# jaymarichua/Applestar

Hardware: AMD Instinct MI355X
Metric: learner samples/sec (AlphaStar policy) (higher is better)
Workload: dtype fp32

## Files before the change

applestar_amd/csrc/bindings.cpp:

```cpp
#include <cstring>
#include <cstdlib>
#include <map>
#include <string>
#include <torch/extension.h>
#include <c10/hip/HIPStream.h>
#include <c10/hip/HIPGuard.h>

#include "kernels.h"

namespace {

hipStream_t stream() { return c10::hip::getCurrentHIPStream().stream(); }

int dt(const at::Tensor& t) {
  if (t.scalar_type() == at::kFloat) return as::DT_F32;
  if (t.scalar_type() == at::kBFloat16) return as::DT_BF16;
  TORCH_CHECK(false, "applestar_amd: unsupported dtype ", t.scalar_type());
}

void check_cuda(const at::Tensor& t, const char* name) {
  TORCH_CHECK(t.is_cuda(), "applestar_amd: ", name, " must be a GPU tensor");
  TORCH_CHECK(t.is_contiguous(), "applestar_amd: ", name, " must be contiguous");
}

// ... 1467 lines not shown
  }
  c10::hip::HIPGuard g(dy.device().index());
  auto opts = out_bf16 ? dy.options() : dy.options().dtype(at::kFloat);
  auto dw = at::empty({N, K}, opts);
  at::Tensor db = want_bias ? at::empty({N}, opts) : at::Tensor();
  if (R == 0) {
    dw.zero_();
    if (want_bias) db.zero_();
    return {dw, db};
  }
  as::small_tn(dy.data_ptr(), x.data_ptr(), mp, static_cast<int>(mask_mode), dw.data_ptr(),
               want_bias ? db.data_ptr() : nullptr, R, static_cast<int>(N), static_cast<int>(K), bf, out_bf16, stream());
  return {dw, db};
}

std::vector<at::Tensor> wgrad_f32(const at::Tensor& dy, const at::Tensor& x, int64_t cin, bool want_bias,
                                  const c10::optional<at::Tensor>& out) {
  check_cuda(dy, "dy");
  check_cuda(x, "x");
  TORCH_CHECK(dy.scalar_type() == at::kFloat && x.scalar_type() == at::kFloat, "wgrad_f32: fp32 dy / x");
  TORCH_CHECK(dy.dim() == 2 && dy.is_contiguous() && x.is_contiguous(), "wgrad_f32: contiguous dy [R, N], x");
  const int64_t R = dy.size(0), N = dy.size(1);
  int64_t K, H = 1, W = 1;
  if (cin > 0) {
    TORCH_CHECK(x.dim() == 4 && x.size(3) == cin && x.size(0) * x.size(1) * x.size(2) == R, "wgrad_f32: x NHWC");
    H = x.size(1);
    W = x.size(2);
    K = 9 * cin;
    TORCH_CHECK(cin % 4 == 0, "wgrad_f32: Cin % 4");
  } else {
    TORCH_CHECK(x.dim() == 2 && x.size(0) == R, "wgrad_f32: x [R, K]");
    K = x.size(1);
  }
  TORCH_CHECK(N % 4 == 0 && K % 4 == 0, "wgrad_f32: N and K must be multiples of 4");
  TORCH_CHECK(R * N * 4 < 0x7ffffff0LL && x.numel() * 4 < 0x7ffffff0LL, "wgrad_f32: tensor too large");
  c10::hip::HIPGuard g(dy.device().index());
  auto opts = dy.options();
  const int64_t NK = N * K, stride = NK + (want_bias ? N : 0);
  at::Tensor flat;
  if (out && out->defined()) {
    TORCH_CHECK(out->scalar_type() == at::kFloat && out->is_contiguous() && out->numel() == stride &&
                out->device() == dy.device(), "wgrad_f32: out must be a contiguous fp32 [N K (+ N)] buffer");
    flat = *out;
  }
  if (R == 0) {
    if (flat.defined()) {
      flat.zero_();
      return {flat.narrow(0, 0, NK).view({N, K}), want_bias ? flat.narrow(0, NK, N) : at::Tensor()};
    }
    return {at::zeros({N, K}, opts), want_bias ? at::zeros({N}, opts) : at::Tensor()};
  }
  const int S = cin > 0 ? as::conv_wgrad_f32_splits(R, static_cast<int>(N), static_cast<int>(K), static_cast<int>(H),
                                                    static_cast<int>(W), static_cast<int>(cin))
                        : as::wgrad_f32_splits(R, static_cast<int>(N), static_cast<int>(K));
  auto part = (S == 1 && flat.defined()) ? flat.view({1, stride}) : at::empty({S, stride}, opts);
  as::wgrad_f32(dy.data_ptr<float>(), x.data_ptr<float>(), part.data_ptr<float>(),
                want_bias ? part.data_ptr<float>() + NK : nullptr, stride, R, static_cast<int>(N), static_cast<int>(K),
                static_cast<int>(H), static_cast<int>(W), static_cast<int>(cin), S, stream());
  if (S == 1) {
    if (!flat.defined()) flat = part.view({stride});
  } else {
    if (!flat.defined()) flat = at::empty({stride}, opts);
    as::column_reduce(part.data_ptr<float>(), flat.data_ptr<float>(), S, static_cast<int>(stride), stream());
  }
  return {flat.narrow(0, 0, NK).view({N, K}), want_bias ? flat.narrow(0, NK, N) : at::Tensor()};
}

std::vector<at::Tensor> wgrad(const at::Tensor& dy, const at::Tensor& x, int64_t cin, bool want_bias, bool bf16_out) {
  check_cuda(dy, "dy");
  check_cuda(x, "x");
  TORCH_CHECK(dy.scalar_type() == at::kBFloat16 && x.scalar_type() == at::kBFloat16, "wgrad: bf16 dy / x");
  TORCH_CHECK(dy.dim() == 2, "wgrad: dy [R, N]");
  TORCH_CHECK(dy.is_contiguous() && x.is_contiguous(), "wgrad: dy and x must be contiguous");
  const int64_t R = dy.size(0), N = dy.size(1);
  int64_t K, H = 1, W = 1;
  if (cin > 0) {
    TORCH_CHECK(x.dim() == 4 && x.size(3) == cin && x.size(0) * x.size(1) * x.size(2) == R, "wgrad: x NHWC");
    H = x.size(1);
    W = x.size(2);
    K = 9 * cin;
    TORCH_CHECK(cin % 8 == 0, "wgrad: Cin % 8");
  } else {
    TORCH_CHECK(x.dim() == 2 && x.size(0) == R, "wgrad: x [R, K]");
    K = x.size(1);
  }
  TORCH_CHECK(N % 8 == 0 && K % 8 == 0, "wgrad: N and K must be multiples of 8");
  TORCH_CHECK(R * N * 2 < 0x7ffffff0LL && x.numel() * 2 < 0x7ffffff0LL, "wgrad: tensor too large");
  c10::hip::HIPGuard g(dy.device().index());
  const int S = R > 0 ? as::wgrad_splits(R, static_cast<int>(N), static_cast<int>(K)) : 1;
  auto opts = dy.options().dtype(at::kFloat);
  if (R == 0) {
    auto zo = bf16_out ? dy.options() : opts;
    return {at::zeros({N, K}, zo), want_bias ? at::zeros({N}, zo) : at::Tensor()};
  }
  const int64_t NK = N * K, stride = NK + (want_bias ? N : 0);
  if (bf16_out && S == 1) {
    auto flat = at::empty({stride}, dy.options());
    as::wgrad(dy.data_ptr(), x.data_ptr(), reinterpret_cast<float*>(flat.data_ptr()),
              want_bias ? reinterpret_cast<float*>(static_cast<at::BFloat16*>(flat.data_ptr()) + NK) : nullptr, 0, R,
              static_cast<int>(N), static_cast<int>(K), static_cast<int>(H), static_cast<int>(W), static_cast<int>(cin),
              1, stream(), true);
    return {flat.narrow(0, 0, NK).view({N, K}), want_bias ? flat.narrow(0, NK, N) : at::Tensor()};
  }
  auto part = at::empty({S, stride}, opts);
  static const bool nan_fill = [] {
    const char* e = std::getenv("APPLESTAR_WGRAD_NANFILL");
    return e != nullptr && e[0] == '1';
// ... 758 lines not shown
  }
  flush();
}

at::Tensor pointwise_conv(const at::Tensor& x, const at::Tensor& w, const c10::optional<at::Tensor>& bias, int64_t act) {
  check_cuda(x, "x");
  check_cuda(w, "w");
  TORCH_CHECK(x.scalar_type() == at::kBFloat16 && x.dim() == 2, "pointwise: x [P, cin] bf16");
  TORCH_CHECK(w.scalar_type() == at::kFloat && w.dim() == 2 && w.size(1) == x.size(1), "pointwise: w fp32 [cout, cin]");
  const int64_t P = x.size(0), cin = x.size(1), cout = w.size(0);
  TORCH_CHECK(as::pointwise_supported(static_cast<int>(cin), static_cast<int>(cout)), "pointwise: channels");
  const float* bp = nullptr;
  if (bias.has_value()) {
    check_cuda(*bias, "bias");
    TORCH_CHECK(bias->scalar_type() == at::kFloat && bias->numel() == cout, "pointwise: bias fp32 [cout]");
    bp = bias->data_ptr<float>();
  }
  c10::hip::HIPGuard g(x.device().index());
  auto y = at::empty({P, cout}, x.options());
  as::pointwise_conv(x.data_ptr(), w.data_ptr<float>(), bp, y.data_ptr(), P, static_cast<int>(cin),
                     static_cast<int>(cout), static_cast<int>(act), stream());
  return y;
}

void register_codec(pybind11::module& m);

PYBIND11_MODULE(TORCH_EXTENSION_NAME, m) {
  m.doc() = "applestar_amd HIP kernels for gfx950 (MI355X)";
  register_codec(m);
  m.def("layer_norm_fwd", &layer_norm_fwd);
  m.def("layer_norm_bwd", &layer_norm_bwd, py::arg("dy"), py::arg("xin"), py::arg("y"), py::arg("w"), py::arg("mean"),
        py::arg("rstd"), py::arg("dx_dtype"), py::arg("act"), py::arg("mask_src") = py::none());
  m.def("reverse_scan", &reverse_scan);
  m.def("col_sum", &col_sum);
  m.def("multi_logp", &multi_logp);
  m.def("presplit_b", &presplit_b, py::arg("b"), py::arg("trans") = false, py::arg("out") = py::none());
  m.def("gemm_f32_psb_supported", &gemm_f32_psb_supported);
  m.def("multi_presplit", &multi_presplit);
  m.def("conv3x3_f32_psb_supported", &conv3x3_f32_psb_supported);
  m.def("conv3x3_f32_psb", &conv3x3_f32_psb, py::arg("x"), py::arg("wsplit"), py::arg("Cout"),
        py::arg("bias") = py::none(), py::arg("res") = py::none(), py::arg("res2") = py::none(),
        py::arg("mask") = py::none(), py::arg("act") = 0);
  m.def("conv3x3_f32_v2", &conv3x3_f32_v2, py::arg("x"), py::arg("wsplit"), py::arg("Cout"),
        py::arg("bias") = py::none(), py::arg("res") = py::none(), py::arg("res2") = py::none(),
        py::arg("mask") = py::none(), py::arg("act") = 0, py::arg("variant") = 0);
  m.def("conv3x3_f32_halo_supported", &conv3x3_f32_halo_supported);
  m.def("conv3x3_f32_halo", &conv3x3_f32_halo, py::arg("x"), py::arg("wsplit"), py::arg("Cout"),
        py::arg("bias") = py::none(), py::arg("res") = py::none(), py::arg("res2") = py::none(),
        py::arg("mask") = py::none(), py::arg("act") = 0);
  m.def("conv_halo_f32_mode", &as::conv_halo_f32_mode);
  m.def("set_conv_halo_f32_mode", &as::set_conv_halo_f32_mode);
  m.def("conv_wgrad_halo_f32_mode", &as::conv_wgrad_halo_f32_mode);
  m.def("set_conv_wgrad_halo_f32_mode", &as::set_conv_wgrad_halo_f32_mode);
  m.def("conv_wgrad_f32_halo_selected", &as::conv_wgrad_f32_halo_selected, py::arg("cout"), py::arg("h"), py::arg("w"),
        py::arg("cin"));
  m.def("gemm_f32_psb", &gemm_f32_psb, py::arg("a"), py::arg("bsplit"), py::arg("N"), py::arg("K"),
        py::arg("bias") = py::none(), py::arg("res") = py::none(), py::arg("act") = 0, py::arg("variant") = 0);
  m.def("entity_pack", &entity_pack);
  m.def("embed_relu_fwd", &embed_relu_fwd);
  m.def("embed_relu_bwd", &embed_relu_bwd, py::arg("dout"), py::arg("out"), py::arg("idx"), py::arg("V"),
        py::arg("ordered") = false);
  m.def("gated_residual_fwd", &gated_residual_fwd, py::arg("y"), py::arg("g"), py::arg("sp"), py::arg("x"),
        py::arg("post") = py::none());
  m.def("gated_residual_bwd", &gated_residual_bwd, py::arg("dout"), py::arg("y"), py::arg("g"), py::arg("sp"),
        py::arg("out"), py::arg("xin") = py::none());
  m.def("lnlstm_fwd", &lnlstm_fwd, py::arg("xp"), py::arg("h0"), py::arg("c0"), py::arg("wT"),
        py::arg("lnh_w"), py::arg("lnh_b"), py::arg("lnc_w"), py::arg("lnc_b"),
        py::arg("eps"), py::arg("want_bf16") = false);
  m.def("lnlstm_bwd", &lnlstm_bwd);
  m.def("entity_embed_fwd", &entity_embed_fwd);
  m.def("entity_onehot", &entity_onehot);
  m.def("upsample2x_fwd", &upsample2x_fwd);
  m.def("upsample2x_bwd", &upsample2x_bwd, py::arg("dy"), py::arg("mask") = py::none());
  m.def("entity_embed_wgrad", &entity_embed_wgrad);
  m.def("mm_k32", &mm_k32);
  m.def("spatial_embed_fwd", &spatial_embed_fwd, py::arg("planes"), py::arg("effects"), py::arg("w_dense"),
        py::arg("bias"), py::arg("rows"), py::arg("ex"), py::arg("ey"), py::arg("entity_num"), py::arg("out_dtype"),
        py::arg("ordered") = false);
  m.def("spatial_gather_rows", &spatial_gather_rows, py::arg("dpre"), py::arg("ex"), py::arg("ey"),
        py::arg("entity_num"), py::arg("N"), py::arg("gate") = py::none());
  m.def("spatial_dense_input", &spatial_dense_input);
  m.def("spatial_dense_wgrad", &spatial_dense_wgrad, py::arg("planes"), py::arg("effects"), py::arg("dpre"),
        py::arg("gate") = py::none());
  m.def("varlen_attn_fwd", &varlen_attn_fwd);
  m.def("varlen_attn_bwd", &varlen_attn_bwd);
  m.def("varlen_attn_fwd_f32", &varlen_attn_fwd_f32);
  m.def("conv3x3_f32_epi2", &conv3x3_f32_epi2);
  m.def("conv3x3_f32_epi2_supported", &conv3x3_f32_epi2_supported);
  m.def("conv3x3_f32", &conv3x3_f32);
  m.def("fused_clip_adam", &fused_clip_adam);
  m.def("head_sample", &head_sample);
  m.def("target_unit_sample", &target_unit_sample);
  m.def("fused_adam_chunk", &as::fused_adam_chunk);
  m.def("wgrad_f32", &wgrad_f32, py::arg("dy"), py::arg("x"), py::arg("cin"), py::arg("want_bias"),
        py::arg("out") = py::none());
  m.def("gemm_f32", &gemm_f32);
  m.def("gemm_bf16_small", &gemm_bf16_small);
  m.def("gemm_bf16", &gemm_bf16);
  m.def("small_gemm", &small_gemm);
  m.def("small_wgrad", &small_wgrad);
  m.def("small_gemm_splitk", &small_gemm_splitk);
  m.def("f32_mfma_mode", &as::f32_mfma_mode);
  m.def("set_f32_pipe_variant", &as::set_f32_pipe_variant);
  m.def("set_f32_conv_variant", &as::set_f32_conv_variant);
  m.def("set_f32_mfma_mode", &as::set_f32_mfma_mode);
  m.def("conv3x3_f32_supported", &as::conv3x3_f32_supported);
// ... 61 lines not shown
```

applestar_amd/csrc/kernels.h:

```cpp
#pragma once
#include <hip/hip_runtime.h>
#include <stdint.h>

namespace as {

enum DType : int { DT_F32 = 0, DT_BF16 = 1 };
enum SrcType : int { SRC_U8 = 0, SRC_I8 = 1, SRC_I16 = 2, SRC_I32 = 3, SRC_I64 = 4, SRC_F16 = 5, SRC_F32 = 6 };
enum FieldKind : int { FIELD_ONE_HOT = 0, FIELD_BINARY = 1, FIELD_SCALAR = 2 };

constexpr int kMaxFields = 40;
struct EntityFields {
  const void* ptr[kMaxFields];
  int dtype[kMaxFields];
  int kind[kMaxFields];
  int offset[kMaxFields];
  int width[kMaxFields];
  int n;
};

void layer_norm_fwd(const void* x, int x_dt, const void* res, int res_dt, const float* w, const float* b,
                    void* y, int y_dt, float* xsum, float* mean, float* rstd, long rows, int cols, float eps,
                    int act, hipStream_t s);
void layer_norm_bwd(const void* dy, int dy_dt, const void* xin, int xin_dt, const void* y, int y_dt,
                    const float* w, const float* mean, const float* rstd, void* dx, int dx_dt,
// ... 127 lines not shown

namespace as {
void maxpool2_fwd(const void* x, void* y, uint8_t* pos, int dt, int B, int H, int W, int C, hipStream_t s);
void maxpool2_bwd(const void* dy, const uint8_t* pos, void* dx, int dt, int B, int H, int W, int C, hipStream_t s,
                  const void* mask = nullptr);
void maxpool2_bwd_relu(const void* dy, const uint8_t* pos, const void* y, void* dx, int B, int H, int W, int C,
                       hipStream_t s, bool f32 = false);
void segment_sum(const void* x, int dt, const int* cu, float* out, int S, int C, hipStream_t s);
void entity_mean_pool(const void* x, int dt, const bool* valid, const void* num, bool num64, void* out, int B, int N,
                      int C, hipStream_t s);
int ln_affine_slices(long R);
void ln_affine_grads(const float* dy, const float* xh, float* part, long R, int C, hipStream_t s);
void table_grad(const void* src, int dt, const int64_t* idx, float* out, long U, int V, int D, hipStream_t s);

bool conv3x3_supported(int Cin, int Cout);
void conv3x3_fwd(const void* x, const void* w, const float* bias, const void* res, void* out, int B, int H, int W,
                 int Cin, int Cout, int act, hipStream_t s);

bool conv3x3_f32_supported(int Cin, int Cout);
void conv3x3_f32_fwd(const float* x, const float* w, const float* bias, const float* res, float* out, int B, int H,
                     int W, int Cin, int Cout, int act, hipStream_t s);
bool conv3x3_f32_epi2_supported(int Cin, int Cout);
void conv3x3_f32_fwd_epi2(const float* x, const float* w, const float* res, const float* res2, long res2_rows,
                          const float* mask, float* out, int B, int H, int W, int Cin, int Cout, hipStream_t s);
int wgrad_f32_splits(long R, int N, int K);
void set_f32_pipe_variant(int v);
int f32_conv_variant();
void set_f32_conv_variant(int v);
int f32_mfma_mode();
void set_f32_mfma_mode(int mode);
void small_nt(const void* a, const void* b, const float* bias, const void* res, const void* amask, int mask_mode,
              void* out, long M, int N, int K, int act, bool bf16, hipStream_t s);
int small_nt_splits(long M, int N, int K);
void small_nt_splitk(const void* a, const void* b, const float* bias, float* part, int S, void* out, long M, int N,
                     int K, int act, bool bf16, hipStream_t s);
void small_tn(const void* dy, const void* x, const void* ymask, int mask_mode, void* dw, void* db, long R, int N,
              int K, bool bf16_in, bool bf16_out, hipStream_t s);
void gemm_bf16_small(const void* a, const void* b, const float* bias, const void* res, void* out, long M, int N, int K,
                     int act, hipStream_t s);
bool gemm_f32_is_small(long M, int N);
void gemm_bf16(const void* a, const void* b, const float* bias, const void* res, void* out, long M, int N, int K,
               int act, hipStream_t s);
void gemm_f32(const float* a, const float* b, const float* bias, const float* res, float* out, long M, int N, int K,
              int act, hipStream_t s);
void wgrad_f32(const float* dy, const float* x, float* dw_part, float* db_part, long part_stride, long R, int N, int K,
               int H, int W, int Cin, int S, hipStream_t st);
int conv_wgrad_halo_f32_mode();
void set_conv_wgrad_halo_f32_mode(int mode);
bool conv_wgrad_f32_halo_supported(int N, int H, int W, int Cin);
bool conv_wgrad_f32_halo_selected(int N, int H, int W, int Cin);
int conv_wgrad_f32_splits(long R, int N, int K, int H, int W, int Cin);
void conv_wgrad_f32_halo(const float* dy, const float* x, float* dw_part, float* db_part, long part_stride, long R,
                         int N, int K, int H, int W, int Cin, int S, long rows_per_split, hipStream_t st);

void head_sample(const void* logits, int logits_dt, long ld_logits, int B, int C, float inv_t, const uint8_t* mask,
                 long mask_ld, const int64_t* lens, const float* u, const void* table, int table_dt,
                 const float* tbias, int D, float* out_logits, int64_t* action, float* emb, hipStream_t s);
void target_unit_sample(const void* e, int e_dt, const float* w1, const float* b1, const float* w2, const float* b2,
                        const void* key, int key_dt, int B, int N, const int64_t* lens, float inv_t, const float* u,
                        float* out_logits, int64_t* action, hipStream_t s);

int fused_adam_chunk();
void fused_clip_adam(const void* table, const long* chunks, int nchunks, int ntensors, float* part,
                     const float* gate, float* norm_out, float max_norm, float* mom, float* scale, float* mom_init,
                     const float* hp, float lr_bc1, float b1, float b2, float inv_sqrt_bc2, float eps, float wd,
                     int decoupled, hipStream_t s);

int wgrad_splits(long R, int N, int K);

constexpr int kCopyMaxT = 64;
constexpr long kCopyChunk = 8192;
constexpr long kCopyRawChunk = 16384;
struct CopyArgs {
  int ntensors;
  int chunk_start[kCopyMaxT + 1];
  const void* src[kCopyMaxT];
  void* dst[kCopyMaxT];
  long n[kCopyMaxT];
  unsigned char dts[kCopyMaxT];
};
void multi_copy(const CopyArgs& a, hipStream_t s);

constexpr int kColMaxP = 32;
struct ColSumArgs {
  int npieces;
  long rows;
  int block_start[kColMaxP + 1];
  float* dst[kColMaxP];
  int dld[kColMaxP], doff[kColMaxP], width[kColMaxP], nsrc[kColMaxP];
  const float* src[kColMaxP][3];
  int sld[kColMaxP][3], soff[kColMaxP][3];
};
void col_sum(const ColSumArgs& a, hipStream_t s);

constexpr int kLogpMaxH = 8;
struct LogpArgs {
  int nheads;
  long row_start[kLogpMaxH + 1];
  const void* logits[kLogpMaxH];
  const int64_t* action[kLogpMaxH];
  float* out[kLogpMaxH];
  int cols[kLogpMaxH];
  unsigned char bf16[kLogpMaxH];
  long blk_start[kLogpMaxH + 1];
  unsigned char big[kLogpMaxH];
};
// ... 170 lines not shown
```

applestar_amd/csrc/kernels/conv_wgrad_f32_halo.hip:

```cpp
#include <cstdlib>

#include "../common.h"
#include "../kernels.h"
#include "../split_mfma.h"
#include "../f32_pipe.h"
#include "../conv_tap.h"

namespace as {
namespace {

using pipe::f16v;

constexpr int kWgBN = 128, kWgCC = 32, kWgRS = 16, kWgMaxW = 80;

typedef short s16x4 __attribute__((ext_vector_type(4)));
typedef __attribute__((address_space(3))) s16x4 lds_s16x4;

template <int WMAX>
struct WgHaloCfg {
  static constexpr int SA = kWgBN * 2 + 64, SX = kWgCC * 2;
  static constexpr int NRING = 2 * kWgRS + 2 * WMAX + 2 <= 128 ? 128 : 256;
  static constexpr int PA = kWgRS * SA;
  static constexpr int PX = (NRING + 1) * SX;
  static constexpr int SMEM = 6 * PA + 3 * PX;
  static_assert(2 * kWgRS + 2 * WMAX + 2 <= NRING && 2 * SMEM <= 160 * 1024, "ring size / two workgroups per CU");
};

__device__ __forceinline__ s16x4 tr_read(const char* p) {
  return __builtin_amdgcn_ds_read_tr16_b64_v4i16((lds_s16x4*)p);
}

__device__ __forceinline__ u32v4 tr_frag(const char* p0, const char* p1) {
  const uint2 lo = __builtin_bit_cast(uint2, tr_read(p0)), hi = __builtin_bit_cast(uint2, tr_read(p1));
  return u32v4{lo.x, lo.y, hi.x, hi.y};
}

__device__ __forceinline__ void split_store(char* plane0, int plane_bytes, int off, const uint4 v) {
  uint2 s0, s1, s2;
  split4(v, s0, s1, s2);
  *reinterpret_cast<uint2*>(plane0 + off) = s0;
  *reinterpret_cast<uint2*>(plane0 + plane_bytes + off) = s1;
  *reinterpret_cast<uint2*>(plane0 + 2 * plane_bytes + off) = s2;
}

template <int WMAX>
__global__ __launch_bounds__(256, 2) void conv_wgrad_f32_halo_kernel(const float* __restrict__ dy,
                                                                     const float* __restrict__ x,
                                                                     float* __restrict__ dw_part,
                                                                     float* __restrict__ db_part, long part_stride,
                                                                     long R, int N, int K, int H, int W, int Cin,
                                                                     long rows_per_split, int tiles_n, int chunks) {
  using C = WgHaloCfg<WMAX>;
  constexpr int RS = kWgRS, BN = kWgBN, CC = kWgCC, SA = C::SA, SX = C::SX;
  constexpr int RINGB = C::NRING * SX;
  __shared__ __attribute__((aligned(16))) char smem[C::SMEM];
  char* const pa = smem;
  char* const px = smem + 6 * C::PA;

  const int wg = pipe::xcd_remap();
  const int ch = wg % chunks;
  const int tn = (wg / chunks) % tiles_n;
  const int s = wg / (chunks * tiles_n);
  const int n0 = tn * BN, c0 = ch * CC;
  const long r_begin = static_cast<long>(s) * rows_per_split;
  const long r_end = r_begin + rows_per_split < R ? r_begin + rows_per_split : R;
  const int tid = threadIdx.x, lane = tid & 63, wid = __builtin_amdgcn_readfirstlane(tid >> 6);
  const int l32 = lane & 31, h = lane >> 5;
  const int HW = H * W;
  const __amdgpu_buffer_rsrc_t yr =
      __builtin_amdgcn_make_buffer_rsrc(const_cast<float*>(dy), 0, static_cast<int>(R * N * 4), 0x00020000);
  const __amdgpu_buffer_rsrc_t xr =
      __builtin_amdgcn_make_buffer_rsrc(const_cast<float*>(x), 0, static_cast<int>(R * Cin * 4), 0x00020000);
  const int nrows = r_end > r_begin ? static_cast<int>(r_end - r_begin) : 0;
  const int nsteps = (nrows + RS - 1) / RS;

  const int a_q = tid & 31, a_row = tid >> 5;
  const bool a_colok = n0 + 4 * a_q < N;
  int a_base[2], a_lim[2];
#pragma unroll
  for (int i = 0; i < 2; ++i) {
    a_base[i] = static_cast<int>(((r_begin + a_row + 8 * i) * N + n0 + 4 * a_q) * 4);
    a_lim[i] = a_colok ? nrows - (a_row + 8 * i) : 0;
  }
  const int a_step = RS * N * 4;
  const int x_q = tid & 7, x_row = (tid >> 3) & 15;
  const bool x_colok = c0 + 4 * x_q < Cin, x_wave = wid < 2;
  const int x_base = static_cast<int>(((r_begin + W + 1 + x_row) * Cin + c0 + 4 * x_q) * 4);
  const long x_left = R - (r_begin + W + 1 + x_row);
  const int x_lim = (x_colok && x_wave && x_left > 0) ? static_cast<int>(x_left) : 0;
  const int x_step = RS * Cin * 4;
  const bool do_bias = db_part != nullptr && ch == 0;
  const int b_col = n0 + (tid & 127), b_h = tid >> 7;
  const int b_base = static_cast<int>(((r_begin + 8 * b_h) * N + b_col) * 4);
  const int b_lim = b_col < N ? nrows - 8 * b_h : 0;
  float rb[8], bsum = 0.f;
  uint4 ra[2], rx;
// ... 432 lines not shown
```

applestar_amd/csrc/kernels/wgrad_f32.hip:

```cpp
#include "../common.h"
#include "../kernels.h"
#include "../split_mfma.h"
#include "../f32_pipe.h"

namespace as {
namespace {

typedef __attribute__((ext_vector_type(16))) float f16v;

template <int BN_, int BK_>
struct WgF32Cfg {
  static constexpr int BN = BN_, BK = BK_, BR = 32, NT = 256;
  static constexpr int WN = BN_ >= 64 ? 2 : 1, WK = 4 / WN;
  static constexpr int TN = BN / WN, TK = BK / WK;
  static constexpr int FN = TN / 32, FK = TK / 32;
  static constexpr int PA = BN + 4, PB = BK + 4;
  static constexpr int CHA = BN / 4, CHB = BK / 4;
  static constexpr int A_IT = BR * CHA / NT, B_IT = BR * CHB / NT;
  static constexpr int STAGE = BR * (PA + PB);
  static_assert(A_IT * NT == BR * CHA && B_IT * NT == BR * CHB, "tile / thread mismatch");
};

template <int BN, int BK, bool CONV, int SPLIT>
__global__ __launch_bounds__(256) void wgrad_f32_kernel(const float* __restrict__ dy, const float* __restrict__ x,
// ... 147 lines not shown
#pragma unroll
      for (int i = 0; i < C::FN; ++i)
#pragma unroll
        for (int j = 0; j < C::FK; ++j)
          acc[i][j] = __builtin_amdgcn_mfma_f32_32x32x2f32(af[i], bfr[j], acc[i][j], 0, 0, 0);
      if (do_bias) {
#pragma unroll
        for (int i = 0; i < C::FN; ++i) bsum[i] += af[i];
      }
    }
    }
    if (it + 1 < nsteps) store_lds(cur ^ 1);
    __syncthreads();
  }

  float* outp = dw_part + static_cast<long>(s) * part_stride;
#pragma unroll
  for (int i = 0; i < C::FN; ++i)
#pragma unroll
    for (int j = 0; j < C::FK; ++j) {
      const int k = k0 + wk * C::TK + 32 * j + l32;
      if (k >= K) continue;
#pragma unroll
      for (int e = 0; e < 16; ++e) {
        const int n = n0 + wn * C::TN + 32 * i + (e & 3) + 8 * (e >> 2) + 4 * h;
        if (n < N) outp[static_cast<long>(n) * K + k] = acc[i][j][e];
      }
    }
  if (do_bias) {
#pragma unroll
    for (int i = 0; i < C::FN; ++i) {
      const float v = bsum[i] + __shfl_xor(bsum[i], 32, kWave);
      const int n = n0 + wn * C::TN + 32 * i + l32;
      if (h == 0 && n < N) db_part[static_cast<long>(s) * part_stride + n] = v;
    }
  }
}

template <int BN, int BK, bool CONV, int NS>
__global__ __launch_bounds__(256, ((BN == 128 && BK >= 128) || BN == 32) ? 2 : 3) void wgrad_f32_pipe_kernel(const float* __restrict__ dy,
                                                                const float* __restrict__ x,
                                                                float* __restrict__ dw_part, float* __restrict__ db_part,
                                                                long part_stride, long R, int N, int K, int H, int W,
                                                                int Cin, long rows_per_split, int tiles_n, int tiles_k) {
  constexpr int RS = BN == 32 ? 32 : 16, SUB = RS / 16;
  constexpr int A_BYTES = RS * BN * 4, B_BYTES = RS * BK * 4, STAGE = A_BYTES + B_BYTES;
  constexpr int A_PW = A_BYTES / 4096, B_PW = B_BYTES / 4096;
  constexpr int A_CPR = BN / 4, B_CPR = BK / 4;
  constexpr int A_RPI = 64 / A_CPR, B_RPI = 64 / B_CPR;
  static_assert(A_PW >= 1 && B_PW >= 1 && A_PW * 4096 == A_BYTES && B_PW * 4096 == B_BYTES, "tile / DMA mismatch");
  constexpr int WN = BN >= 64 ? 2 : 1, WK = 4 / WN;
  constexpr int TN = BN / WN, TK = BK / WK, FN = TN / 32, FK = TK / 32;
  static_assert(NS == 3, "three stage arrays");
  __shared__ __attribute__((aligned(16))) char s0[STAGE], s1[STAGE], s2[STAGE];
  char* const smem[3] = {s0, s1, s2};

  const int wg = pipe::xcd_remap();
  const int tk = wg % tiles_k;
  const int tn = (wg / tiles_k) % tiles_n;
  const int s = wg / (tiles_k * tiles_n);
  const int n0 = tn * BN, k0 = tk * BK;
  const long r_begin = static_cast<long>(s) * rows_per_split;
  const long r_end = r_begin + rows_per_split < R ? r_begin + rows_per_split : R;
  const int tid = threadIdx.x, lane = tid & 63, wid = __builtin_amdgcn_readfirstlane(tid >> 6);
  const int wn = wid / WK, wk = wid % WK;
  const int l32 = lane & 31, h = lane >> 5;
  const long HW = static_cast<long>(H) * W;
  const pipe::i32x4 yr = pipe::rsrc(dy, R * N * 4), xr = pipe::rsrc(x, CONV ? R * Cin * 4 : R * K * 4);

  const int a_col = n0 + 4 * (lane % A_CPR), b_col = k0 + 4 * (lane % B_CPR);
  int a_row[A_PW], b_row[B_PW];
#pragma unroll
  for (int c = 0; c < A_PW; ++c) a_row[c] = (wid + 4 * c) * A_RPI + lane / A_CPR;
#pragma unroll
  for (int c = 0; c < B_PW; ++c) b_row[c] = (wid + 4 * c) * B_RPI + lane / B_CPR;
  int b_c = b_col, b_dy = 0, b_dx = 0;
  if (CONV) {
    const int tap = b_col / Cin;
    b_c = b_col - tap * Cin;
    b_dy = tap / 3 - 1;
    b_dx = tap % 3 - 1;
  }
  const bool a_ok = a_col < N, b_ok = b_col < K;
  int py[B_PW], px[B_PW];
  const int adv_y = RS / W, adv_x = RS % W;
  if (CONV) {
#pragma unroll
    for (int c = 0; c < B_PW; ++c) {
      const int rem = static_cast<int>((r_begin + b_row[c]) % HW);
      py[c] = rem / W;
      px[c] = rem - py[c] * W;
    }
  }
  const long nsteps = r_end > r_begin ? (r_end - r_begin + RS - 1) / RS : 0;
  auto issue = [&](char* st, long kt) {
    const long r0 = r_begin + kt * RS;
#pragma unroll
    for (int c = 0; c < A_PW; ++c) {
      const long r = r0 + a_row[c];
      pipe::dma16(yr, st + (wid + 4 * c) * 1024,
                  (kt < nsteps && a_ok && r < r_end) ? (static_cast<int>(r) * N + a_col) * 4 : pipe::kOOB);
    }
#pragma unroll
    for (int c = 0; c < B_PW; ++c) {
      const long r = r0 + b_row[c];
      int off = pipe::kOOB;
      if (CONV) {
        const int yy = py[c] + b_dy, xx = px[c] + b_dx;
        if (kt < nsteps && b_ok && r < r_end && yy >= 0 && yy < H && xx >= 0 && xx < W)
          off = ((static_cast<int>(r) + b_dy * W + b_dx) * Cin + b_c) * 4;
        px[c] += adv_x;
        py[c] += adv_y;
        if (px[c] >= W) { px[c] -= W; ++py[c]; }
        while (py[c] >= H) py[c] -= H;
      } else if (kt < nsteps && b_ok && r < r_end) {
        off = (static_cast<int>(r) * K + b_col) * 4;
      }
      pipe::dma16(xr, st + A_BYTES + (wid + 4 * c) * 1024, off);
    }
  };

  f16v acc[FN][FK];
#pragma unroll
  for (int i = 0; i < FN; ++i)
#pragma unroll
    for (int j = 0; j < FK; ++j)
#pragma unroll
      for (int e = 0; e < 16; ++e) acc[i][j][e] = 0.f;
  const bool do_bias = db_part != nullptr && tk == 0 && wk == 0;
  float bsum[FN];
#pragma unroll
  for (int i = 0; i < FN; ++i) bsum[i] = 0.f;

  auto step = [&](const char* st, char* next, long kt) {
    pipe::wait_vm<(NS - 2) * (A_PW + B_PW)>();
    __builtin_amdgcn_s_barrier();
    asm volatile("" ::: "memory");
    issue(next, kt + NS - 1);
#pragma unroll
    for (int sub = 0; sub < SUB; ++sub) {
      const float* A = reinterpret_cast<const float*>(st) + (16 * sub + 8 * h) * BN + wn * TN + l32;
      const float* Bt = reinterpret_cast<const float*>(st + A_BYTES) + (16 * sub + 8 * h) * BK + wk * TK + l32;
      float av[FN][8];
#pragma unroll
      for (int t = 0; t < 8; ++t)
#pragma unroll
        for (int i = 0; i < FN; ++i) av[i][t] = A[t * BN + 32 * i];
      Split3 sa[FN];
#pragma unroll
      for (int i = 0; i < FN; ++i) sa[i] = split8(av[i]);
      if constexpr (FK <= 2) {
        float bv[FK][8];
#pragma unroll
        for (int t = 0; t < 8; ++t)
#pragma unroll
          for (int j = 0; j < FK; ++j) bv[j][t] = Bt[t * BK + 32 * j];
        Split3 sb[FK];
#pragma unroll
        for (int j = 0; j < FK; ++j) sb[j] = split8(bv[j]);
#pragma unroll
        for (int i = 0; i < FN; ++i)
#pragma unroll
          for (int j = 0; j < FK; ++j) acc[i][j] = mfma_x6(sa[i], sb[j], acc[i][j]);
      } else {
#pragma unroll
        for (int j = 0; j < FK; ++j) {
          float bv[8];
#pragma unroll
          for (int t = 0; t < 8; ++t) bv[t] = Bt[t * BK + 32 * j];
          const Split3 sb = split8(bv);
#pragma unroll
          for (int i = 0; i < FN; ++i) acc[i][j] = mfma_x6(sa[i], sb, acc[i][j]);
        }
      }
      if (do_bias) {
#pragma unroll
        for (int i = 0; i < FN; ++i)
#pragma unroll
          for (int t = 0; t < 8; ++t) bsum[i] += av[i][t];
      }
    }
  };
  issue(smem[0], 0);
  issue(smem[1], 1);
  for (long kt = 0; kt < nsteps; kt += NS) {
    step(smem[0], smem[2], kt);
    if (kt + 1 >= nsteps) break;
    step(smem[1], smem[0], kt + 1);
    if (kt + 2 >= nsteps) break;
    step(smem[2], smem[1], kt + 2);
  }
  pipe::wait_vm<0>();

  float* outp = dw_part + static_cast<long>(s) * part_stride;
#pragma unroll
  for (int i = 0; i < FN; ++i)
#pragma unroll
    for (int j = 0; j < FK; ++j) {
      const int k = k0 + wk * TK + 32 * j + l32;
      if (k >= K) continue;
#pragma unroll
      for (int e = 0; e < 16; ++e) {
        const int n = n0 + wn * TN + 32 * i + (e & 3) + 8 * (e >> 2) + 4 * h;
        if (n < N) outp[static_cast<long>(n) * K + k] = acc[i][j][e];
      }
    }
  if (do_bias) {
#pragma unroll
    for (int i = 0; i < FN; ++i) {
      const float v = bsum[i] + __shfl_xor(bsum[i], 32, kWave);
      const int n = n0 + wn * TN + 32 * i + l32;
      if (h == 0 && n < N) db_part[static_cast<long>(s) * part_stride + n] = v;
    }
  }
}

template <int BN>
struct StgCfg {
  static constexpr int BK = 128, RS = 16;
  static constexpr int WN = BN == 128 ? 2 : 1, WK = 4 / WN;
  static constexpr int FN = BN / (32 * WN), FK = BK / (32 * WK);
  static constexpr int A_BYTES = RS * BN * 4, B_BYTES = RS * BK * 4, FST = A_BYTES + B_BYTES;
  static constexpr int A_N = A_BYTES / 1024, B_N = B_BYTES / 1024;
  static constexpr int A_PW = (A_N + 3) / 4, B_PW = B_N / 4;
  static constexpr int A_CPR = BN / 4, B_CPR = BK / 4, A_RPI = 64 / A_CPR, B_RPI = 64 / B_CPR;
  static constexpr int PLA = (BN / 32) * 2 * 32 * 16, PLB = (BK / 32) * 2 * 32 * 16;
  static constexpr int PST = 3 * (PLA + PLB);
// ... 165 lines not shown
      const int k = k0 + wk * 32 * FK + 32 * j + l32;
      if (k >= K) continue;
#pragma unroll
      for (int e = 0; e < 16; ++e) {
        const int n = n0 + wn * 32 * FN + 32 * i + (e & 3) + 8 * (e >> 2) + 4 * h;
        if (n < N) outp[static_cast<long>(n) * K + k] = acc[i][j][e];
      }
    }
  if (do_bias) {
    float* bred = reinterpret_cast<float*>(F);
    __syncthreads();
    if (a_split && ah == 1) bred[ac] = bsum;
    __syncthreads();
    if (a_split && ah == 0 && n0 + ac < N) db_part[static_cast<long>(s) * part_stride + n0 + ac] = bsum + bred[ac];
  }
}

bool wgrad_f32_pipe32_off() {
  static const bool off = [] {
    const char* e = std::getenv("APPLESTAR_WGRAD32_PIPE");
    return e == nullptr || e[0] != '1';
  }();
  return off;
}

bool wgrad_stg() {
  static const bool on = [] {
    const char* e = std::getenv("APPLESTAR_WGRAD_STG");
    return e == nullptr || e[0] != '0';
  }();
  return on;
}

bool wgrad_stg_narrow() {
  static const bool on = [] {
    const char* e = std::getenv("APPLESTAR_WGRAD_STG_NARROW");
    return e != nullptr && e[0] == '1';
  }();
  return on;
}

template <int BN, int BK, bool CONV>
void launch(const float* dy, const float* x, float* dwp, float* dbp, long ps, long R, int N, int K, int H, int W,
            int Cin, int S, long rps, hipStream_t st) {
  const int tn = (N + BN - 1) / BN, tk = (K + BK - 1) / BK;
  const long nwg = static_cast<long>(tn) * tk * S;
  if constexpr (BK == 128) {
    if (f32_mfma_mode() == 1 && wgrad_stg() && (BN == 128 || wgrad_stg_narrow())) {
      hipLaunchKernelGGL((wgrad_f32_stg_kernel<BN, CONV>), dim3(static_cast<unsigned>(nwg)), dim3(256), 0, st, dy, x,
                         dwp, dbp, ps, R, N, K, H, W, Cin, rps, tn, tk);
      return;
    }
  }
  if constexpr (BN >= 32 && (BK <= 128 || (BN == 128 && BK == 256))) {
    if (f32_mfma_mode() == 1 && !(BN == 32 && wgrad_f32_pipe32_off())) {
      hipLaunchKernelGGL((wgrad_f32_pipe_kernel<BN, BK, CONV, 3>), dim3(static_cast<unsigned>(nwg)), dim3(256), 0, st,
                         dy, x, dwp, dbp, ps, R, N, K, H, W, Cin, rps, tn, tk);
      return;
    }
  }
  if (f32_mfma_mode())
    hipLaunchKernelGGL((wgrad_f32_kernel<BN, BK, CONV, 1>), dim3(static_cast<unsigned>(nwg)), dim3(256), 0, st, dy, x,
                       dwp, dbp, ps, R, N, K, H, W, Cin, rps, tn, tk);
  else
    hipLaunchKernelGGL((wgrad_f32_kernel<BN, BK, CONV, 0>), dim3(static_cast<unsigned>(nwg)), dim3(256), 0, st, dy,
                       x, dwp, dbp, ps, R, N, K, H, W, Cin, rps, tn, tk);
}

int pick(int n) { return n <= 32 ? 32 : (n <= 64 ? 64 : 128); }
bool wgrad32_bk256() {
  static const bool on = [] {
    const char* e = std::getenv("APPLESTAR_WGRAD32_BK");
    return e != nullptr && e[0] == '2';
  }();
  return on;
}
bool wgrad_wide() {
  static const bool on = [] {
    const char* e = std::getenv("APPLESTAR_WGRAD_WIDE");
    return e != nullptr && e[0] == '1';
  }();
  return on;
}
int pick_k(int k, int bn) {
  if (bn == 32) return (k >= 256 && wgrad32_bk256()) ? 256 : 128;
  if (bn == 128 && k >= 256 && wgrad_wide() && f32_mfma_mode() == 1) return 256;
  return k <= 64 ? 64 : 128;
}

}

long wgrad_f32_target_wg() {
  static const long v = [] {
    const char* e = std::getenv("APPLESTAR_WGRAD_F32_WG");
    const long x = e ? std::atol(e) : 3072;
    return x >= 64 ? x : 3072;
  }();
  return v;
}

long wgrad_f32_small_r_rows() {
  static const long v = [] {
    const char* e = std::getenv("APPLESTAR_WGRAD_SMALL_R");
    return e ? std::atol(e) : 48L;
  }();
  return v;
}

int wgrad_f32_splits(long R, int N, int K) {
  const int bn = pick(N), bk = pick_k(K, bn);
  const long tiles = static_cast<long>((N + bn - 1) / bn) * ((K + bk - 1) / bk);
  const long target = wgrad_f32_target_wg();
  long S = (target + tiles - 1) / tiles;
  const long small = wgrad_f32_small_r_rows();
  const long max_s = R < 2048 ? (small > 0 && R >= 2 * small ? R / small : 1)
                              : (R + 127) / 128;
  if (S > max_s) S = max_s;
  const long max_part = (16L << 20) / (static_cast<long>(N) * K);
  if (S > max_part) S = max_part;
  if (S < 1) S = 1;
  if (S > 4096) S = 4096;
  return static_cast<int>(S);
}

void wgrad_f32(const float* dy, const float* x, float* dw_part, float* db_part, long part_stride, long R, int N, int K,
               int H, int W, int Cin, int S, hipStream_t st) {
  long rps = (R + S - 1) / S;
  rps = (rps + 31) / 32 * 32;
  const bool conv = Cin > 0;
  if (conv && conv_wgrad_f32_halo_selected(N, H, W, Cin)) {
    conv_wgrad_f32_halo(dy, x, dw_part, db_part, part_stride, R, N, K, H, W, Cin, S, rps, st);
    return;
  }
  const int bn = pick(N), bk = pick_k(K, bn);
#define AS_WGF(BNv, BKv)                                                                   \
  if (bn == BNv && bk == BKv) {                                                            \
    if (conv) launch<BNv, BKv, true>(dy, x, dw_part, db_part, part_stride, R, N, K, H, W, Cin, S, rps, st); \
    else launch<BNv, BKv, false>(dy, x, dw_part, db_part, part_stride, R, N, K, H, W, Cin, S, rps, st);     \
    return;                                                                                \
  }
  AS_WGF(128, 128) AS_WGF(128, 64) AS_WGF(64, 128) AS_WGF(64, 64) AS_WGF(32, 128) AS_WGF(32, 256) AS_WGF(128, 256)
#undef AS_WGF
}

}
```

Before: 8366.

## Add wide-tile dense fp32 wgrad kernel with pre-split LDS planes and transpose reads

Adds a dedicated dense (non-conv) fp32 weight-gradient kernel that uses 128x256 tiles. It converts dy and x into three split planes in LDS at store time and reads MFMA fragments with ds_read_tr transposed loads, double-buffered across row steps. The kernel has its own split-count heuristic with a lower workgroup target. By default it is enabled for large R, N>64, K>=256 when K is a multiple of 256 or the last chunk is more than half of 256. The goal is more reuse of the dy tile per workgroup and less register-side splitting. The old opt-in BK=256 pipe path is removed, and the shared transpose helpers move into a common header.

```diff
diff --git a/applestar_amd/csrc/bindings.cpp b/applestar_amd/csrc/bindings.cpp
--- a/applestar_amd/csrc/bindings.cpp
+++ b/applestar_amd/csrc/bindings.cpp
@@ -1543,7 +1543,7 @@
   }
   const int S = cin > 0 ? as::conv_wgrad_f32_splits(R, static_cast<int>(N), static_cast<int>(K), static_cast<int>(H),
                                                     static_cast<int>(W), static_cast<int>(cin))
-                        : as::wgrad_f32_splits(R, static_cast<int>(N), static_cast<int>(K));
+                        : as::dense_wgrad_f32_splits(R, static_cast<int>(N), static_cast<int>(K));
   auto part = (S == 1 && flat.defined()) ? flat.view({1, stride}) : at::empty({S, stride}, opts);
   as::wgrad_f32(dy.data_ptr<float>(), x.data_ptr<float>(), part.data_ptr<float>(),
                 want_bias ? part.data_ptr<float>() + NK : nullptr, stride, R, static_cast<int>(N), static_cast<int>(K),
@@ -2408,6 +2408,9 @@
   m.def("set_conv_halo_f32_mode", &as::set_conv_halo_f32_mode);
   m.def("conv_wgrad_halo_f32_mode", &as::conv_wgrad_halo_f32_mode);
   m.def("set_conv_wgrad_halo_f32_mode", &as::set_conv_wgrad_halo_f32_mode);
+  m.def("dense_wgrad_wide_f32_mode", &as::dense_wgrad_wide_f32_mode);
+  m.def("set_dense_wgrad_wide_f32_mode", &as::set_dense_wgrad_wide_f32_mode);
+  m.def("dense_wgrad_f32_wide_selected", &as::dense_wgrad_f32_wide_selected, py::arg("r"), py::arg("n"), py::arg("k"));
   m.def("conv_wgrad_f32_halo_selected", &as::conv_wgrad_f32_halo_selected, py::arg("cout"), py::arg("h"), py::arg("w"),
         py::arg("cin"));
   m.def("gemm_f32_psb", &gemm_f32_psb, py::arg("a"), py::arg("bsplit"), py::arg("N"), py::arg("K"),
diff --git a/applestar_amd/csrc/kernels.h b/applestar_amd/csrc/kernels.h
--- a/applestar_amd/csrc/kernels.h
+++ b/applestar_amd/csrc/kernels.h
@@ -203,6 +203,12 @@
 int conv_wgrad_f32_splits(long R, int N, int K, int H, int W, int Cin);
 void conv_wgrad_f32_halo(const float* dy, const float* x, float* dw_part, float* db_part, long part_stride, long R,
                          int N, int K, int H, int W, int Cin, int S, long rows_per_split, hipStream_t st);
+int dense_wgrad_wide_f32_mode();
+void set_dense_wgrad_wide_f32_mode(int mode);
+bool dense_wgrad_f32_wide_selected(long R, int N, int K);
+int dense_wgrad_f32_splits(long R, int N, int K);
+void dense_wgrad_f32_wide(const float* dy, const float* x, float* dw_part, float* db_part, long part_stride, long R,
+                          int N, int K, int S, long rows_per_split, hipStream_t st);
 
 void head_sample(const void* logits, int logits_dt, long ld_logits, int B, int C, float inv_t, const uint8_t* mask,
                  long mask_ld, const int64_t* lens, const float* u, const void* table, int table_dt,
diff --git a/applestar_amd/csrc/kernels/conv_wgrad_f32_halo.hip b/applestar_amd/csrc/kernels/conv_wgrad_f32_halo.hip
--- a/applestar_amd/csrc/kernels/conv_wgrad_f32_halo.hip
+++ b/applestar_amd/csrc/kernels/conv_wgrad_f32_halo.hip
@@ -5,6 +5,7 @@
 #include "../split_mfma.h"
 #include "../f32_pipe.h"
 #include "../conv_tap.h"
+#include "../wgrad_tr.h"
 
 namespace as {
 namespace {
@@ -12,9 +13,6 @@
 using pipe::f16v;
 
 constexpr int kWgBN = 128, kWgCC = 32, kWgRS = 16, kWgMaxW = 80;
-
-typedef short s16x4 __attribute__((ext_vector_type(4)));
-typedef __attribute__((address_space(3))) s16x4 lds_s16x4;
 
 template <int WMAX>
 struct WgHaloCfg {
@@ -25,23 +23,6 @@
   static constexpr int SMEM = 6 * PA + 3 * PX;
   static_assert(2 * kWgRS + 2 * WMAX + 2 <= NRING && 2 * SMEM <= 160 * 1024, "ring size / two workgroups per CU");
 };
-
-__device__ __forceinline__ s16x4 tr_read(const char* p) {
-  return __builtin_amdgcn_ds_read_tr16_b64_v4i16((lds_s16x4*)p);
-}
-
-__device__ __forceinline__ u32v4 tr_frag(const char* p0, const char* p1) {
-  const uint2 lo = __builtin_bit_cast(uint2, tr_read(p0)), hi = __builtin_bit_cast(uint2, tr_read(p1));
-  return u32v4{lo.x, lo.y, hi.x, hi.y};
-}
-
-__device__ __forceinline__ void split_store(char* plane0, int plane_bytes, int off, const uint4 v) {
-  uint2 s0, s1, s2;
-  split4(v, s0, s1, s2);
-  *reinterpret_cast<uint2*>(plane0 + off) = s0;
-  *reinterpret_cast<uint2*>(plane0 + plane_bytes + off) = s1;
-  *reinterpret_cast<uint2*>(plane0 + 2 * plane_bytes + off) = s2;
-}
 
 template <int WMAX>
 __global__ __launch_bounds__(256, 2) void conv_wgrad_f32_halo_kernel(const float* __restrict__ dy,
diff --git a/applestar_amd/csrc/kernels/dense_wgrad_f32.hip b/applestar_amd/csrc/kernels/dense_wgrad_f32.hip
--- /dev/null
+++ b/applestar_amd/csrc/kernels/dense_wgrad_f32.hip
@@ -0,0 +1,225 @@
+#include <cstdlib>
+#include <type_traits>
+
+#include "../common.h"
+#include "../kernels.h"
+#include "../split_mfma.h"
+#include "../f32_pipe.h"
+#include "../wgrad_tr.h"
+
+namespace as {
+namespace {
+
+using pipe::f16v;
+
+constexpr int kDwBN = 128, kDwBK = 256, kDwRS = 16, kDwNB = kDwBK / 32;
+constexpr int kDwSA = kDwBN * 2 + 64, kDwSX = 64;
+constexpr int kDwPA = kDwRS * kDwSA;
+constexpr int kDwXB = kDwRS * kDwSX;
+constexpr int kDwPX = kDwNB * kDwXB;
+constexpr int kDwSMEM = 6 * kDwPA + 6 * kDwPX;
+static_assert(2 * kDwSMEM <= 160 * 1024, "two workgroups per CU");
+static_assert(8 * kDwBN * 4 <= kDwSMEM, "the db sums reuse the planes");
+
+__global__ __launch_bounds__(256, 2) void dense_wgrad_f32_kernel(const float* __restrict__ dy,
+                                                                 const float* __restrict__ x,
+                                                                 float* __restrict__ dw_part,
+                                                                 float* __restrict__ db_part, long part_stride,
+                                                                 long R, int N, int K, long rows_per_split,
+                                                                 int tiles_n, int chunks) {
+  constexpr int RS = kDwRS, BN = kDwBN, BK = kDwBK, SA = kDwSA, SX = kDwSX, PA = kDwPA, PX = kDwPX, XB = kDwXB;
+  __shared__ __attribute__((aligned(16))) char smem[kDwSMEM];
+  char* const pa = smem;
+  char* const px = smem + 6 * PA;
+
+  const int wg = pipe::xcd_remap();
+  const int ch = wg % chunks;
+  const int tn = (wg / chunks) % tiles_n;
+  const int s = wg / (chunks * tiles_n);
+  const int n0 = tn * BN, k0 = ch * BK;
+  const long r_begin = static_cast<long>(s) * rows_per_split;
+  const long r_end = r_begin + rows_per_split < R ? r_begin + rows_per_split : R;
+  const int tid = threadIdx.x, lane = tid & 63, wid = __builtin_amdgcn_readfirstlane(tid >> 6);
+  const int l32 = lane & 31, h = lane >> 5;
+  const __amdgpu_buffer_rsrc_t yr =
+      __builtin_amdgcn_make_buffer_rsrc(const_cast<float*>(dy), 0, static_cast<int>(R * N * 4), 0x00020000);
+  const __amdgpu_buffer_rsrc_t xr =
+      __builtin_amdgcn_make_buffer_rsrc(const_cast<float*>(x), 0, static_cast<int>(R * K * 4), 0x00020000);
+  const int nrows = r_end > r_begin ? static_cast<int>(r_end - r_begin) : 0;
+  const int nsteps = (nrows + RS - 1) / RS;
+  const bool half = K - k0 <= BK / 2;
+
+  const int a_q = tid & 31, a_row = tid >> 5;
+  const bool a_colok = n0 + 4 * a_q < N;
+  int a_base[2], a_lim[2];
+#pragma unroll
+  for (int i = 0; i < 2; ++i) {
+    a_base[i] = static_cast<int>(((r_begin + a_row + 8 * i) * N + n0 + 4 * a_q) * 4);
+    a_lim[i] = a_colok ? nrows - (a_row + 8 * i) : 0;
+  }
+  const int a_step = RS * N * 4;
+  const int x_q = tid & 7, x_row = (tid >> 3) & 15, x_b0 = tid >> 7;
+  const int x_base = static_cast<int>(((r_begin + x_row) * K + k0 + 32 * x_b0 + 4 * x_q) * 4);
+  int x_lim[4];
+#pragma unroll
+  for (int i = 0; i < 4; ++i) x_lim[i] = k0 + 32 * (x_b0 + 2 * i) + 4 * x_q < K ? nrows - x_row : 0;
+  const int x_step = RS * K * 4;
+  const bool do_bias = db_part != nullptr && ch == 0;
+  float bs[4] = {0.f, 0.f, 0.f, 0.f};
+  const int a_dst = a_row * SA + a_q * 8;
+  const int x_dst = x_b0 * XB + x_row * SX + x_q * 8;
+
+  const int g = lane >> 4, tq = (lane >> 2) & 3, tp = lane & 3;
+  const int rr0 = 8 * (g >> 1) + tq;
+  const int a_off = rr0 * SA + (32 * wid + 16 * (g & 1) + 4 * tp) * 2;
+  const int x_off = rr0 * SX + (16 * (g & 1) + 4 * tp) * 2;
+
+  f16v acc[kDwNB];
+#pragma unroll
+  for (int b = 0; b < kDwNB; ++b)
+#pragma unroll
+    for (int e = 0; e < 16; ++e) acc[b][e] = 0.f;
+
+  auto run = [&](auto nbc) {
+    constexpr int NB = decltype(nbc)::value, XP = NB / 2;
+    uint4 ra[2], rx[XP];
+    auto load_stage = [&](int j) {
+#pragma unroll
+      for (int i = 0; i < 2; ++i) {
+        const auto v =
+            __builtin_amdgcn_raw_buffer_load_b128(yr, j * RS < a_lim[i] ? a_base[i] + j * a_step : kOOB, 0, 0);
+        ra[i] = make_uint4(v[0], v[1], v[2], v[3]);
+      }
+#pragma unroll
+      for (int i = 0; i < XP; ++i) {
+        const auto v = __builtin_amdgcn_raw_buffer_load_b128(
+            xr, j * RS < x_lim[i] ? x_base + j * x_step + i * 256 : kOOB, 0, 0);
+        rx[i] = make_uint4(v[0], v[1], v[2], v[3]);
+      }
+    };
+    auto store_stage = [&](int j) {
+      char* const da = pa + (j & 1) * 3 * PA;
+      char* const dx = px + (j & 1) * 3 * PX;
+#pragma unroll
+      for (int i = 0; i < 2; ++i) {
+        split_store(da, PA, a_dst + 8 * i * SA, ra[i]);
+        if (do_bias) {
+          bs[0] += __uint_as_float(ra[i].x);
+          bs[1] += __uint_as_float(ra[i].y);
+          bs[2] += __uint_as_float(ra[i].z);
+          bs[3] += __uint_as_float(ra[i].w);
+        }
+      }
+#pragma unroll
+      for (int i = 0; i < XP; ++i) split_store(dx, PX, x_dst + 2 * i * XB, rx[i]);
+    };
+
+    load_stage(0);
+    store_stage(0);
+    __syncthreads();
+    for (int j = 0; j < nsteps; ++j) {
+      const bool more = j + 1 < nsteps;
+      if (more) load_stage(j + 1);
+      const char* ap = pa + (j & 1) * 3 * PA + a_off;
+      Split3 fa;
+#pragma unroll
+      for (int p = 0; p < 3; ++p) fa.p[p] = tr_frag(ap + p * PA, ap + p * PA + 4 * SA);
+      const char* xp = px + (j & 1) * 3 * PX + x_off;
+      auto read_x = [&](int b) {
+        Split3 f;
+#pragma unroll
+        for (int p = 0; p < 3; ++p) f.p[p] = tr_frag(xp + p * PX + b * XB, xp + p * PX + b * XB + 4 * SX);
+        return f;
+      };
+      Split3 fb[2];
+      fb[0] = read_x(0);
+#pragma unroll
+      for (int b = 0; b < NB; ++b) {
+        if (b + 1 < NB) fb[(b + 1) & 1] = read_x(b + 1);
+        __builtin_amdgcn_sched_barrier(0);
+        acc[b] = mfma_x6(fa, fb[b & 1], acc[b]);
+        __builtin_amdgcn_sched_barrier(0);
+      }
+      if (more) store_stage(j + 1);
+      __syncthreads();
+    }
+  };
+  if (half) run(std::integral_constant<int, kDwNB / 2>{});
+  else run(std::integral_constant<int, kDwNB>{});
+
+  float* outp = dw_part + static_cast<long>(s) * part_stride;
+#pragma unroll
+  for (int b = 0; b < kDwNB; ++b) {
+    const int k = k0 + 32 * b + l32;
+    if (k < K) {
+#pragma unroll
+      for (int e = 0; e < 16; ++e) {
+        const int n = n0 + 32 * wid + (e & 3) + 8 * (e >> 2) + 4 * h;
+        if (n < N) outp[static_cast<long>(n) * K + k] = acc[b][e];
+      }
+    }
+  }
+  if (do_bias) {
+    float* const red = reinterpret_cast<float*>(smem);
+#pragma unroll
+    for (int q = 0; q < 4; ++q) red[a_row * BN + 4 * a_q + q] = bs[q];
+    __syncthreads();
+    if (tid < BN && n0 + tid < N) {
+      float v = red[tid];
+      for (int i = 1; i < 8; ++i) v += red[i * BN + tid];
+      db_part[static_cast<long>(s) * part_stride + n0 + tid] = v;
+    }
+  }
+}
+
+int& dw_wide_ref() {
+  static int v = [] {
+    const char* e = std::getenv("APPLESTAR_DENSE_WGRAD_WIDE_F32");
+    return e ? std::atoi(e) & 7 : 5;
+  }();
+  return v;
+}
+
+long dw_wide_target() {
+  static const long v = [] {
+    const char* e = std::getenv("APPLESTAR_DENSE_WGRAD_WIDE_WG");
+    const long x = e ? std::atol(e) : 512;
+    return x >= 1 ? x : 512;
+  }();
+  return v;
+}
+
+}
+
+int dense_wgrad_wide_f32_mode() { return dw_wide_ref(); }
+void set_dense_wgrad_wide_f32_mode(int mode) { dw_wide_ref() = mode & 7; }
+
+bool dense_wgrad_f32_wide_selected(long R, int N, int K) {
+  if (f32_mfma_mode() != 1 || R < 2048 || N <= 64 || K < 256) return false;
+  const int rem = K % kDwBK;
+  const int bit = rem == 0 ? 1 : (rem <= kDwBK / 2 ? 2 : 4);
+  return (dense_wgrad_wide_f32_mode() & bit) != 0;
+}
+
+int dense_wgrad_f32_splits(long R, int N, int K) {
+  if (!dense_wgrad_f32_wide_selected(R, N, K)) return wgrad_f32_splits(R, N, K);
+  const long tiles = static_cast<long>((N + kDwBN - 1) / kDwBN) * ((K + kDwBK - 1) / kDwBK);
+  long S = dw_wide_target() / tiles;
+  const long max_s = (R + 2 * kDwRS - 1) / (2 * kDwRS);
+  if (S > max_s) S = max_s;
+  const long max_part = (16L << 20) / (static_cast<long>(N) * K);
+  if (S > max_part) S = max_part;
+  if (S < 1) S = 1;
+  if (S > 4096) S = 4096;
+  return static_cast<int>(S);
+}
+
+void dense_wgrad_f32_wide(const float* dy, const float* x, float* dw_part, float* db_part, long part_stride, long R,
+                          int N, int K, int S, long rows_per_split, hipStream_t st) {
+  const int tiles_n = (N + kDwBN - 1) / kDwBN, chunks = (K + kDwBK - 1) / kDwBK;
+  const long nwg = static_cast<long>(S) * tiles_n * chunks;
+  hipLaunchKernelGGL(dense_wgrad_f32_kernel, dim3(static_cast<unsigned>(nwg)), dim3(256), 0, st, dy, x, dw_part,
+                     db_part, part_stride, R, N, K, rows_per_split, tiles_n, chunks);
+}
+
+}
diff --git a/applestar_amd/csrc/kernels/wgrad_f32.hip b/applestar_amd/csrc/kernels/wgrad_f32.hip
--- a/applestar_amd/csrc/kernels/wgrad_f32.hip
+++ b/applestar_amd/csrc/kernels/wgrad_f32.hip
@@ -223,6 +223,7 @@
   constexpr int WN = BN >= 64 ? 2 : 1, WK = 4 / WN;
   constexpr int TN = BN / WN, TK = BK / WK, FN = TN / 32, FK = TK / 32;
   static_assert(NS == 3, "three stage arrays");
+  static_assert(FK <= 2, "at most two X fragments per wave");
   __shared__ __attribute__((aligned(16))) char s0[STAGE], s1[STAGE], s2[STAGE];
   char* const smem[3] = {s0, s1, s2};
 
@@ -320,30 +321,18 @@
       Split3 sa[FN];
 #pragma unroll
       for (int i = 0; i < FN; ++i) sa[i] = split8(av[i]);
-      if constexpr (FK <= 2) {
-        float bv[FK][8];
-#pragma unroll
-        for (int t = 0; t < 8; ++t)
-#pragma unroll
-          for (int j = 0; j < FK; ++j) bv[j][t] = Bt[t * BK + 32 * j];
-        Split3 sb[FK];
-#pragma unroll
-        for (int j = 0; j < FK; ++j) sb[j] = split8(bv[j]);
-#pragma unroll
-        for (int i = 0; i < FN; ++i)
-#pragma unroll
-          for (int j = 0; j < FK; ++j) acc[i][j] = mfma_x6(sa[i], sb[j], acc[i][j]);
-      } else {
-#pragma unroll
-        for (int j = 0; j < FK; ++j) {
-          float bv[8];
-#pragma unroll
-          for (int t = 0; t < 8; ++t) bv[t] = Bt[t * BK + 32 * j];
-          const Split3 sb = split8(bv);
-#pragma unroll
-          for (int i = 0; i < FN; ++i) acc[i][j] = mfma_x6(sa[i], sb, acc[i][j]);
-        }
-      }
+      float bv[FK][8];
+#pragma unroll
+      for (int t = 0; t < 8; ++t)
+#pragma unroll
+        for (int j = 0; j < FK; ++j) bv[j][t] = Bt[t * BK + 32 * j];
+      Split3 sb[FK];
+#pragma unroll
+      for (int j = 0; j < FK; ++j) sb[j] = split8(bv[j]);
+#pragma unroll
+      for (int i = 0; i < FN; ++i)
+#pragma unroll
+        for (int j = 0; j < FK; ++j) acc[i][j] = mfma_x6(sa[i], sb[j], acc[i][j]);
       if (do_bias) {
 #pragma unroll
         for (int i = 0; i < FN; ++i)
@@ -615,7 +604,7 @@
       return;
     }
   }
-  if constexpr (BN >= 32 && (BK <= 128 || (BN == 128 && BK == 256))) {
+  if constexpr (BN >= 32 && BK <= 128) {
     if (f32_mfma_mode() == 1 && !(BN == 32 && wgrad_f32_pipe32_off())) {
       hipLaunchKernelGGL((wgrad_f32_pipe_kernel<BN, BK, CONV, 3>), dim3(static_cast<unsigned>(nwg)), dim3(256), 0, st,
                          dy, x, dwp, dbp, ps, R, N, K, H, W, Cin, rps, tn, tk);
@@ -638,16 +627,8 @@
   }();
   return on;
 }
-bool wgrad_wide() {
-  static const bool on = [] {
-    const char* e = std::getenv("APPLESTAR_WGRAD_WIDE");
-    return e != nullptr && e[0] == '1';
-  }();
-  return on;
-}
 int pick_k(int k, int bn) {
   if (bn == 32) return (k >= 256 && wgrad32_bk256()) ? 256 : 128;
-  if (bn == 128 && k >= 256 && wgrad_wide() && f32_mfma_mode() == 1) return 256;
   return k <= 64 ? 64 : 128;
 }
 
@@ -695,6 +676,10 @@
     conv_wgrad_f32_halo(dy, x, dw_part, db_part, part_stride, R, N, K, H, W, Cin, S, rps, st);
     return;
   }
+  if (!conv && dense_wgrad_f32_wide_selected(R, N, K)) {
+    dense_wgrad_f32_wide(dy, x, dw_part, db_part, part_stride, R, N, K, S, rps, st);
+    return;
+  }
   const int bn = pick(N), bk = pick_k(K, bn);
 #define AS_WGF(BNv, BKv)                                                                   \
   if (bn == BNv && bk == BKv) {                                                            \
@@ -702,7 +687,7 @@
     else launch<BNv, BKv, false>(dy, x, dw_part, db_part, part_stride, R, N, K, H, W, Cin, S, rps, st);     \
     return;                                                                                \
   }
-  AS_WGF(128, 128) AS_WGF(128, 64) AS_WGF(64, 128) AS_WGF(64, 64) AS_WGF(32, 128) AS_WGF(32, 256) AS_WGF(128, 256)
+  AS_WGF(128, 128) AS_WGF(128, 64) AS_WGF(64, 128) AS_WGF(64, 64) AS_WGF(32, 128) AS_WGF(32, 256)
 #undef AS_WGF
 }
 
diff --git a/applestar_amd/csrc/wgrad_tr.h b/applestar_amd/csrc/wgrad_tr.h
--- /dev/null
+++ b/applestar_amd/csrc/wgrad_tr.h
@@ -0,0 +1,27 @@
+#pragma once
+#include "common.h"
+#include "split_mfma.h"
+
+namespace as {
+
+typedef short s16x4 __attribute__((ext_vector_type(4)));
+typedef __attribute__((address_space(3))) s16x4 lds_s16x4;
+
+__device__ __forceinline__ s16x4 tr_read(const char* p) {
+  return __builtin_amdgcn_ds_read_tr16_b64_v4i16((lds_s16x4*)p);
+}
+
+__device__ __forceinline__ u32v4 tr_frag(const char* p0, const char* p1) {
+  const uint2 lo = __builtin_bit_cast(uint2, tr_read(p0)), hi = __builtin_bit_cast(uint2, tr_read(p1));
+  return u32v4{lo.x, lo.y, hi.x, hi.y};
+}
+
+__device__ __forceinline__ void split_store(char* plane0, int plane_bytes, int off, const uint4 v) {
+  uint2 s0, s1, s2;
+  split4(v, s0, s1, s2);
+  *reinterpret_cast<uint2*>(plane0 + off) = s0;
+  *reinterpret_cast<uint2*>(plane0 + plane_bytes + off) = s1;
+  *reinterpret_cast<uint2*>(plane0 + 2 * plane_bytes + off) = s2;
+}
+
+}
```

Measured after the change: 8440 (median of 6 runs). About the same (+0.9%).
